# chanzuckerberg/saber

Hardware: AMD Instinct MI355X
Metric: EM slices/sec (1024^2, Hiera-L) (higher is better)
Workload: dtype bf16; 1 GPU; 1024x1024 uint16 EM slice -> prep.prepare -> SAM2 AMG (Hiera-L, cfgAMG defaults: npoints=32, crop_n_layers=2 -> 21 crops, 3072 grid prompts + 9216 m2m refinements, multimask) -> dedup/sort -> uint16 label plane; BASELINE configs[1]; weights=seeded synthetic Hiera-L (no checkpoint offline), slices_per_rank=22, engine_handles_per_gpu=2, parallelism=single GPU

## Files before the change

include/saber_amd.h:

```cpp
#ifndef SABER_AMD_H
#define SABER_AMD_H
#include <stdint.h>

#ifdef __cplusplus
extern "C" {
#endif

typedef struct saber_engine saber_engine;

enum saber_status {
    SABER_OK = 0,
    SABER_ERR_INVALID = -1,
    SABER_ERR_STATE = -2,
    SABER_ERR_HIP = -3,
    SABER_ERR_CAPACITY = -4,
    SABER_ERR_RANGE = -5
};

enum saber_dtype { SABER_U16 = 0, SABER_F32 = 1 };

typedef struct saber_amg_params {
    int points_per_side;
    int points_per_batch;
    float pred_iou_thresh;
// ... 55 lines not shown
#define SABER_WEIGHTS_FP8_E4M3 1
#define SABER_WEIGHTS_MXFP8 2
int saber_engine_set_weight_format(saber_engine* e, int format);

#define SABER_PRECISION_BF16 0
#define SABER_PRECISION_EXACT 1
#define SABER_PRECISION_FP16 2
int saber_engine_set_precision(saber_engine* e, int precision);

int saber_engine_check_finite(saber_engine* e, void* stream);

int saber_engine_set_graphs(saber_engine* e, int enable);
int saber_engine_set_encoder_stream(saber_engine* e, void* stream);
int saber_engine_graph_stats(const saber_engine* e, int* captures, int* replays);

int saber_amg_last_syncs(const saber_engine* e);
int saber_engine_set_device_amg(saber_engine* e, int enable);
int saber_engine_set_iou_pruning(saber_engine* e, int enable);
int saber_engine_set_lowres_cleanup(saber_engine* e, int max_hole_area, int max_sprinkle_area);
int saber_engine_set_multipoint(saber_engine* e, int enable);
int saber_amg_last_pruning(const saber_engine* e, int64_t* pruned, int64_t* m2m_candidates);

int saber_label_plane(saber_engine* e, const uint32_t* bits_dev, const int* order_host, int n, int H, int W,
                      uint16_t* plane_dev, void* stream);

struct saber_window_mask;
int saber_place_window_masks(saber_engine* e, const uint32_t* src_dev, int64_t src_words, const struct saber_window_mask* table_host, int n, int H,
                             int W, uint32_t* out_dev, void* stream);
int saber_window_label_stack(saber_engine* e, const uint32_t* src_dev, int64_t src_words, const struct saber_window_mask* table_host, int n, int first,
                             int count, int H, int W, int elem_bytes, void* out_dev, void* stream);
// ... 88 lines not shown
```

saber_amd/_lib.py:

```python
import ctypes as C
import os
import subprocess

_HERE = os.path.dirname(os.path.abspath(__file__))
LIB_PATH = os.path.join(_HERE, "libsaber_amd.so")
CSRC = os.path.join(_HERE, "csrc")


class SaberAmdError(RuntimeError):
    pass


class SaberRangeError(SaberAmdError):
    """SABER_ERR_RANGE: the engine's overflow sentinel found NaN / inf in the 16-bit arithmetic (include/saber_amd.h:
    saber_engine_check_finite) - with fp16 operands, an activation beyond 65 504.  The call's results are invalid."""


SABER_OK, SABER_ERR_INVALID, SABER_ERR_STATE, SABER_ERR_HIP, SABER_ERR_CAPACITY, SABER_ERR_RANGE = 0, -1, -2, -3, -4, -5


def build(verbose: bool = False) -> str:
    r = subprocess.run(["make", "-C", CSRC, "-j8"], capture_output=True, text=True)
    if r.returncode != 0:
        raise SaberAmdError("building libsaber_amd.so failed:\n" + r.stdout[-4000:] + r.stderr[-4000:])
# ... 57 lines not shown
    "saber_decode_prompts": (_i, [_vp, _i, _vp, _vp, _i, _i, _i, _vp, _vp, _vp, _vp, _vp]),
    "saber_amg_generate": (_i, [_vp, _vp, _i, _i, _i, C.POINTER(AmgParams), _vp, _i, C.POINTER(MaskMeta), C.POINTER(_i), _vp]),
    "saber_amg_postprocess_small_regions": (_i, [_vp, _vp, _i, _i, _i, C.POINTER(MaskMeta), _i, _f, _vp, C.POINTER(_i), _vp]),
    "saber_amg_last_syncs": (_i, [_vp]),
    "saber_engine_set_iou_pruning": (_i, [_vp, _i]),
    "saber_engine_set_lowres_cleanup": (_i, [_vp, _i, _i]),
    "saber_engine_set_multipoint": (_i, [_vp, _i]),
    "saber_engine_set_device_amg": (_i, [_vp, _i]),
    "saber_amg_last_pruning": (_i, [_vp, _vp, _vp]),
    "saber_engine_set_graphs": (_i, [_vp, _i]),
    "saber_engine_set_encoder_stream": (_i, [_vp, _vp]),
    "saber_engine_set_weight_format": (_i, [_vp, _i]),
    "saber_engine_set_precision": (_i, [_vp, _i]),
    "saber_engine_check_finite": (_i, [_vp, _vp]),
    "saber_engine_graph_stats": (_i, [_vp, C.POINTER(_i), C.POINTER(_i)]),
    "saber_label_plane": (_i, [_vp, _vp, C.POINTER(_i), _i, _i, _i, _vp, _vp]),
    "saber_mask_pair_intersections": (_i, [_vp, _vp, _i, _i, _i, _vp, _vp]),
    "saber_place_window_masks": (_i, [_vp, _vp, C.c_int64, C.POINTER(WindowMask), _i, _i, _i, _vp, _vp]),
    "saber_window_label_stack": (_i, [_vp, _vp, C.c_int64, C.POINTER(WindowMask), _i, _i, _i, _i, _i, _i, _vp, _vp]),
    "saber_separate_masks": (_i, [_vp, _vp, _i, _i, _i, _i, _vp, C.POINTER(_i), _vp]),
    "saber_cc_chunk_label": (_i, [_vp, _vp, _i, _i, _i, _vp, _vp, _vp]),
    "saber_cc_seam_pairs": (_i, [_vp, _vp, _vp, _i, _i, C.c_uint32, C.c_uint32, _vp, _i, C.POINTER(_i), _vp]),
    "saber_cc_chunk_roots": (_i, [_vp, _vp, _vp, _i, _i, _i, C.c_uint32, _vp, _i, _vp, _i, C.POINTER(_i), _vp]),
    "saber_cc_chunk_finish": (_i, [_vp, _vp, _vp, _i, _i, _i, _vp, _vp, _i, _vp]),
    "saber_smooth_labels": (_i, [_vp, _vp, _i, _i, _i, _i, C.c_double, _vp, C.POINTER(_i), _vp]),
    "saber_smooth_labels_chunk": (_i, [_vp, _vp, _i, _vp, _i, _vp, _i, _i, _i, _i, _i, _i, _vp, _vp, _i, C.c_double, _vp, C.POINTER(_i), _vp]),
    "saber_smooth_radius": (_i, [C.c_int64, C.c_double, C.POINTER(_i)]),
    "saber_label_max": (_i, [_vp, _vp, _i, C.c_int64, C.POINTER(C.c_uint32), _vp]),
    "saber_label_counts": (_i, [_vp, _vp, _i, _i, _i, _i, _i, _vp, _vp]),
    "saber_gaussian_smoothing_3d": (_i, [_vp, _vp, _i, _i, _i, C.c_double, _vp, _vp]),
# ... 128 lines not shown
```

saber_amd/csrc/amg.hip:

```cpp
#include <algorithm>
#include <array>
#include <cmath>
#include <numeric>

#include "common.h"
#include "engine.h"

#define TRY(x) do { int _r = (x); if (_r != SABER_OK) return _r; } while (0)

struct Cand {
    float box[4];
    float iou, stab;
    float pt[2];
    int crop[4];
    int area;
    size_t bits_slot;
};

static std::vector<int> nms_host(const std::vector<Cand>& c, const std::vector<float>& scores, float thr) {
    const int n = (int)c.size();
    std::vector<int> order(n);
    std::iota(order.begin(), order.end(), 0);
    std::stable_sort(order.begin(), order.end(), [&](int a, int b) { return scores[a] > scores[b]; });
    std::vector<char> sup(n, 0);
// ... 207 lines not shown
        h_pts.resize(n_pts * 2);
        std::vector<float> crop_pts_all(n_pts * 2);
        for (const Grp& gr : groups)
            for (int g = 0; g < gr.G; ++g) {
                const auto& box = crops[c0 + gr.ci + g];
                const int cw = box[2] - box[0], chh = box[3] - box[1];
                for (int iy = 0; iy < gr.gn; ++iy)
                    for (int ix = 0; ix < gr.gn; ++ix) {
                        const float px = (float)(grids[gr.layer][ix] * (double)cw), py = (float)(grids[gr.layer][iy] * (double)chh);
                        const size_t k = gr.pt0 + (size_t)g * gr.np + (size_t)iy * gr.gn + ix;
                        crop_pts_all[2 * k] = px; crop_pts_all[2 * k + 1] = py;
                        h_pts[2 * k] = (px / (float)cw) * 1024.0f;
                        h_pts[2 * k + 1] = (py / (float)chh) * 1024.0f;
                    }
            }
        ENG_HIP(e, hipMemcpyAsync(e->amg_pts, h_pts.data(), sizeof(float) * 2 * n_pts, hipMemcpyHostToDevice, s));
        if (prm->use_m2m) {
            h_pts2.resize(n_cand * 2);
            for (size_t k = 0; k < n_pts; ++k)
                for (int m = 0; m < M; ++m) { h_pts2[2 * (k * M + m)] = h_pts[2 * k]; h_pts2[2 * (k * M + m) + 1] = h_pts[2 * k + 1]; }
            ENG_HIP(e, hipMemcpyAsync(e->amg_pts2, h_pts2.data(), sizeof(float) * 2 * n_cand, hipMemcpyHostToDevice, s));
        }
        for (Grp& gr : groups) {
            const int ci = gr.ci, G = gr.G, np = gr.np, nm = gr.nm;
            float* pts1 = e->amg_pts + 2 * gr.pt0;
            float* low1 = e->amg_low1 + gr.pt0 * (first_raw ? 4 : 1) * 65536;
            float* iou1 = e->amg_iou1 + gr.k0;
            TRY(eng_graphed(e, "dec1," + key_of({ci, np, (long long)(uintptr_t)pts1, G * np, prm->multimask_output, (long long)(uintptr_t)low1, (long long)(uintptr_t)iou1}), s,
                            [&]() { return eng_decode_ex(e, ci, np, pts1, nullptr, G * np, prm->multimask_output, nullptr, 0, 0.f, low1, first_raw, iou1, nullptr, nullptr, s); }));
            for (int g = 0; g < G; ++g) e->slot_shared_valid[ci + g] = 1;
            gr.masks = low1; gr.ious = iou1; gr.plane_mode = first_raw ? 1 : 0;
            if (prm->use_m2m) {
                float* pts2 = e->amg_pts2 + 2 * gr.k0;
                float* low2 = e->amg_low2 + gr.k0 * 4 * 65536;
                float* iou2 = e->amg_iou2 + gr.k0;
                int* sel2 = e->amg_sel + gr.k0;
                TRY(eng_graphed(e, "dec2," + key_of({ci, nm, (long long)(uintptr_t)pts2, G * nm, first_raw, (long long)(uintptr_t)low1, (long long)(uintptr_t)low2, (long long)(uintptr_t)iou2, (long long)(uintptr_t)sel2,
                                                     (long long)(e->iou_prune ? std::lround(prm->pred_iou_thresh * 1e6f) + 1 : 0)}), s,
                                [&]() { return eng_decode_ex(e, ci, nm, pts2, nullptr, G * nm, 0, low1, first_raw, 32.0f, low2, 1, iou2, nullptr, sel2, s, prm->pred_iou_thresh); }));
                for (int g = 0; g < G; ++g) e->slot_embb_valid[ci + g] = 1;
                gr.masks = low2; gr.ious = iou2; gr.plane_mode = 2;
            }
        }
        if (use_dev) {
            const float* iou_all = prm->use_m2m ? e->amg_iou2 : e->amg_iou1;
            std::vector<DevCrop> dcs;
            for (const Grp& gr : groups)
                for (int g = 0; g < gr.G; ++g) {
                    const auto& box = crops[c0 + gr.ci + g];
                    dcs.push_back(DevCrop{{box[0], box[1], box[2], box[3]}, (int)(gr.k0 + (size_t)g * gr.nm), gr.nm, (int)(gr.pt0 + (size_t)g * gr.np), M});
                }
            ENG_HIP(e, hipMemcpyAsync(e->amg_crops_dev, dcs.data(), sizeof(DevCrop) * dcs.size(), hipMemcpyHostToDevice, s));
            size_t dc0 = 0;
            for (const Grp& gr : groups) {
// ... 190 lines not shown
```

saber_amd/csrc/engine.h:

```cpp
#pragma once
#include <hip/hip_runtime.h>
#include <algorithm>
#include <functional>
#include <map>
#include <set>
#include <string>
#include <vector>

#include "../../include/saber_amd.h"
#include "kernels.h"

struct BlockSpec { int din, dout, heads, window, q_stride; };

struct HostTensor { std::vector<int64_t> shape; std::vector<float> data; };

struct LinW { const bf16_t* w = nullptr; const float* b = nullptr; int out = 0, in = 0, ldw = 0; const bf16_t* wpk = nullptr; int wpk_n = 0; const float* wf = nullptr;
              const uint8_t* w8 = nullptr; const uint8_t* sw8 = nullptr; int kp8 = 0, sw_rows = 0; };
struct LnW { const float* g = nullptr; const float* b = nullptr; };

struct BlockW { LnW n1, n2; LinW qkv, proj, fc1, fc2, sc; const bf16_t* mlp_pk = nullptr; };

struct AttnW { LinW q, k, v, o; const bf16_t* pe_proj = nullptr; const bf16_t* img_wT = nullptr; };
struct DecLayerW { AttnW self_attn, t2i, i2t; LnW n1, n2, n3, n4; LinW mlp1, mlp2; };

enum { PC_GEMM = 0, PC_HIERA_ATTN, PC_LAYERNORM, PC_DEC_ATTN, PC_ELEMENTWISE, PC_IMAGE, PC_MASK_POST, PC_DEC_T2I, PC_DEC_I2T, PC_DEC_UPSCALE, PC_GEMM_MX, PC_N };
struct ProfRec { int cls; double flops; double bytes; hipEvent_t a, b; };

struct saber_engine {
    int device = 0;
    std::string trunk;
    int max_images = 1, max_prompts = 64;
    std::string err;
    bool finalized = false;
    int weight_format = 0;
    int precision = 0;
    bool op_f16 = false;
    bool keep_f32 = false;
    void* exact_ws = nullptr;
    void* refine_state = nullptr;
    void* labelstats_ws = nullptr;
    void* sr_ws = nullptr; size_t sr_ws_bytes = 0;
// ... 54 lines not shown
    float* embb = nullptr;
    bf16_t* h2_bf = nullptr;
    std::vector<char> slot_embb_valid;
    std::vector<char> slot_valid, slot_shared_valid;

    float *tok_pe = nullptr, *queries = nullptr, *tq = nullptr, *tk = nullptr;
    bf16_t* t_att = nullptr;
    bf16_t* keys_bf = nullptr;
    bf16_t *fold_q = nullptr, *fold_k = nullptr, *fold_v = nullptr;
    float *fold_cb = nullptr, *t2i_part = nullptr, *t2i_ml = nullptr;
    float *masks4 = nullptr, *hyper_out = nullptr, *iou4 = nullptr;
    bf16_t* hyper_pk = nullptr;
    int* counts_ws = nullptr;
    float* dec_out_masks = nullptr;
    float* dec_out_iou = nullptr;

    float* prep_ws = nullptr; size_t prep_ws_elems = 0; unsigned int* prep_minmax = nullptr;

    float *amg_prep = nullptr; size_t amg_prep_elems = 0;
    int* amg_sel = nullptr; bool amg_m2m_sized = false;
    float *amg_pts = nullptr, *amg_low1 = nullptr, *amg_low2 = nullptr, *amg_iou1 = nullptr, *amg_iou2 = nullptr, *amg_pts2 = nullptr;
    size_t amg_prompts_cap = 0, amg_pts_cap = 0;
    uint32_t* amg_bits = nullptr; size_t amg_bits_words = 0;
    uint32_t* amg_crop_bits = nullptr; size_t amg_crop_words = 0;
    MaskStats* amg_stats = nullptr; int* amg_idx = nullptr; size_t amg_stats_cap = 0;
    int* order_dev = nullptr; size_t order_cap = 0;
    void* win_table_dev = nullptr; size_t win_table_cap = 0;

    bool graphs_on = true;
    std::map<std::string, hipGraphExec_t> graphs;
// ... 54 lines not shown
        if (_st != hipSuccess) { cleanup(); return eng_fail((e), SABER_ERR_HIP, std::string(#call) + ": " + hipGetErrorString(_st)); } \
    } while (0)
#define ENG_K(e, call)                                                   \
    do {                                                                 \
        const char* _m = (call);                                         \
        if (_m) return eng_fail((e), SABER_ERR_INVALID, _m);             \
    } while (0)

int eng_graphed(saber_engine* e, const std::string& key, hipStream_t s, const std::function<int()>& body);
void eng_graphs_flush(saber_engine* e);
int eng_encode(saber_engine* e, const float* img_dev, int H, int W, int channels, const int* crops_host, int n, int slot0, hipStream_t s);
int eng_decode(saber_engine* e, int slot, int per_slot, const float* pts_dev, const int* labels_dev, int n, int multimask,
               const float* mask_in_dev, float mask_clamp, float* out_lowres, float* out_iou, float* out_obj, hipStream_t s);
int eng_decode_ex(saber_engine* e, int slot, int per_slot, const float* pts_dev, const int* labels_dev, int n, int multimask,
                  const float* mask_in_dev, int mask_in_raw4, float mask_clamp, float* out_lowres, int out_raw4, float* out_iou, float* out_obj,
                  int* out_sel, hipStream_t s, float prune_iou_thr = 0.f);
int exact_encode_blocks(saber_engine* e, int n, int slot0, hipStream_t s);
int exact_decode_core(saber_engine* e, int slot0, int per_slot, int p_base, const float* pts, const int* labels, int P, const float* mask_in,
                      float mask_clamp, int mask_in_q0, float* out_obj, float* masks4, hipStream_t s, int n_pts = 1);
int exact_chunk_prompts(const saber_engine* e);
void exact_release(saber_engine* e);
struct UpscalePack {
    std::vector<float> w1, b1;
    std::vector<float> w2, b2;
    std::vector<float> w2p;
};
void saber_pack_upscale(const float* w0, const float* b0, const float* w3, const float* b3, UpscalePack* out);
bf16_t saber_host_f2op(float f, bool f16);
template <typename T> int eng_alloc(saber_engine* e, T** p, size_t count);
int eng_alloc_bytes(saber_engine* e, void** p, size_t bytes);
void eng_free(saber_engine* e, void* p);
// ... 10 lines not shown
```

saber_amd/csrc/engine.hip:

```cpp
#include "engine.h"

#include <algorithm>
#include <cmath>
#include <cstring>
#include <functional>
#include <utility>

#include "common.h"

static thread_local std::string g_create_err;

int eng_fail(saber_engine* e, int code, const std::string& msg) {
    if (e) e->err = msg; else g_create_err = msg;
    return code;
}

int eng_alloc_bytes(saber_engine* e, void** p, size_t bytes) {
    *p = nullptr;
    if (bytes == 0) bytes = 16;
    hipError_t st = hipMalloc(p, bytes);
    if (st != hipSuccess) return eng_fail(e, SABER_ERR_HIP, std::string("hipMalloc(") + std::to_string(bytes) + "): " + hipGetErrorString(st));
    e->allocs.push_back(*p);
    return SABER_OK;
}
// ... 106 lines not shown
extern "C" int saber_engine_set_precision(saber_engine* e, int precision) {
    if (!e) return SABER_ERR_INVALID;
    if (precision != SABER_PRECISION_BF16 && precision != SABER_PRECISION_EXACT && precision != SABER_PRECISION_FP16) return eng_fail(e, SABER_ERR_INVALID, "set_precision: unknown precision");
    if (!e->finalized) {
        if (precision == SABER_PRECISION_EXACT) e->keep_f32 = true;
        else e->op_f16 = precision == SABER_PRECISION_FP16;
    } else {
        if (precision == SABER_PRECISION_EXACT && !e->keep_f32)
            return eng_fail(e, SABER_ERR_STATE, "set_precision: the exact mode needs the fp32 weight copies; request it once before saber_engine_finalize");
        if (precision == SABER_PRECISION_FP16 && !e->op_f16)
            return eng_fail(e, SABER_ERR_STATE, "set_precision: this handle was finalized with bf16 weights; choose SABER_PRECISION_FP16 before saber_engine_finalize");
        if (precision == SABER_PRECISION_BF16 && e->op_f16)
            return eng_fail(e, SABER_ERR_STATE, "set_precision: this handle was finalized with fp16 weights; it runs in SABER_PRECISION_FP16 (or EXACT)");
    }
    e->precision = precision;
    return SABER_OK;
}
extern "C" int saber_engine_set_iou_pruning(saber_engine* e, int enable) {
    if (!e) return SABER_ERR_INVALID;
    if ((bool)enable != e->iou_prune) { e->iou_prune = enable != 0; eng_graphs_flush(e); }
    return SABER_OK;
}
extern "C" int saber_engine_set_lowres_cleanup(saber_engine* e, int max_hole_area, int max_sprinkle_area) {
    if (!e) return SABER_ERR_INVALID;
    if (max_hole_area < 0 || max_hole_area > 65535 || max_sprinkle_area < 0 || max_sprinkle_area > 65535)
        return eng_fail(e, SABER_ERR_INVALID, "set_lowres_cleanup: max_hole_area and max_sprinkle_area must be 0 to 65535");
    e->lowres_hole_area = max_hole_area; e->lowres_sprinkle_area = max_sprinkle_area;
    return SABER_OK;
}
extern "C" int saber_engine_set_multipoint(saber_engine* e, int enable) {
    if (!e) return SABER_ERR_INVALID;
    if (enable && e->max_prompts < 2) return eng_fail(e, SABER_ERR_INVALID, "set_multipoint: the 16-token route needs max_prompts >= 2 (chunks of max_prompts / 2 prompts)");
    e->multipoint = enable != 0;
    return SABER_OK;
}
extern "C" int saber_engine_set_encoder_stream(saber_engine* e, void* stream) {
    if (!e) return SABER_ERR_INVALID;
    if ((hipStream_t)stream != e->enc_stream) { eng_graphs_flush(e); e->enc_stream = (hipStream_t)stream; }
    return SABER_OK;
}
extern "C" int saber_engine_set_graphs(saber_engine* e, int enable) {
    if (!e) return SABER_ERR_INVALID;
    e->graphs_on = enable != 0;
    return SABER_OK;
}
extern "C" int saber_engine_graph_stats(const saber_engine* e, int* captures, int* replays) {
    if (!e) return SABER_ERR_INVALID;
    if (captures) *captures = e->graph_captures;
// ... 39 lines not shown
    *out = e;
    return SABER_OK;
}

extern "C" void saber_engine_destroy(saber_engine* e) {
    if (!e) return;
    (void)hipSetDevice(e->device);
    (void)hipDeviceSynchronize();
    for (auto& kv : e->graphs) (void)hipGraphExecDestroy(kv.second);
    exact_release(e);
    refine_release(e);
    if (e->crops_pin) (void)hipHostFree(e->crops_pin);
    for (hipEvent_t ev : e->crops_ev) if (ev) (void)hipEventDestroy(ev);
    for (hipEvent_t ev : e->enc_ev) if (ev) (void)hipEventDestroy(ev);
    for (void* p : e->allocs) (void)hipFree(p);
    delete e;
}

extern "C" const char* saber_last_error(const saber_engine* e) { return e ? e->err.c_str() : g_create_err.c_str(); }

extern "C" int saber_engine_set_weight(saber_engine* e, const char* name, const float* host, const int64_t* shape, int ndim) {
    if (!e) return SABER_ERR_INVALID;
    if (!name || !host || !shape || ndim < 1 || ndim > 4) return eng_fail(e, SABER_ERR_INVALID, "set_weight: bad argument");
    if (e->finalized) return eng_fail(e, SABER_ERR_STATE, "set_weight after finalize");
    HostTensor t;
    int64_t n = 1;
    for (int i = 0; i < ndim; ++i) { if (shape[i] <= 0) return eng_fail(e, SABER_ERR_INVALID, "set_weight: non-positive dim"); t.shape.push_back(shape[i]); n *= shape[i]; }
    t.data.assign(host, host + n);
    e->host_w[name] = std::move(t);
    return SABER_OK;
// ... 547 lines not shown
            GemmParams g;
            g.A = e->dense_pe_bf; g.lda = 256; g.W = w.w; g.ldw = w.ldw; g.w_kpad = 1; g.M = 4096; g.N = 128; g.K = 256; g.Cb = d; g.ldcb = 128;
            if (const char* m = launch_gemm(g, nullptr)) return eng_fail(e, SABER_ERR_INVALID, m);
            a.pe_proj = d;
            return SABER_OK;
        };
        for (int l = 0; l < 2; ++l) {
            TRY(project(e->dl[l].t2i, e->dl[l].t2i.k));
            TRY(project(e->dl[l].i2t, e->dl[l].i2t.q));
        }
        TRY(project(e->final_attn, e->final_attn.k));
    }
    ENG_HIP(e, hipDeviceSynchronize());
    e->host_w.clear();
    e->finalized = true;
    return SABER_OK;
}

void prof_begin(saber_engine* e, int cls, double flops, double bytes, hipStream_t s) {
    if (!e->prof_on) return;
    while (e->ev_pool.size() < e->ev_used + 2) { hipEvent_t ev; if (hipEventCreate(&ev) != hipSuccess) { e->prof_on = false; return; } e->ev_pool.push_back(ev); }
    ProfRec r; r.cls = cls; r.flops = flops; r.bytes = bytes; r.a = e->ev_pool[e->ev_used++]; r.b = e->ev_pool[e->ev_used++];
    (void)hipEventRecord(r.a, s);
    e->prof.push_back(r);
}
void prof_end(saber_engine* e, hipStream_t s) {
    if (!e->prof_on || e->prof.empty()) return;
    (void)hipEventRecord(e->prof.back().b, s);
}
extern "C" int saber_profile_begin(saber_engine* e) {
// ... 374 lines not shown
    return SABER_OK;
}

static int decode_pick_or_select(saber_engine* e, int P, int multimask, float* out_lowres, float* out_iou, float* raw4_out, int* out_sel, const uint8_t* live,
                                 hipStream_t s) {
    float* oi = out_iou ? out_iou : e->dec_out_iou;
    if (raw4_out) {
        ENG_KP(e, PC_ELEMENTWISE, 0.0, 0.0, launch_mask_pick(raw4_out, e->iou4, P, multimask, oi, out_sel, s, live));
        return SABER_OK;
    }
    float* om = out_lowres ? out_lowres : e->dec_out_masks;
    ENG_KP(e, PC_ELEMENTWISE, 0.0, 0.0, launch_mask_select(e->masks4, e->iou4, P, multimask, om, oi, e->counts_ws, s));
    return SABER_OK;
}

static int decode_chunk(saber_engine* e, int slot0, int per_slot, int p_base, const float* pts, const int* labels, int P, int multimask,
                        const float* mask_in, float mask_clamp, float* out_lowres, float* out_iou, float* out_obj, hipStream_t s,
                        float* raw4_out = nullptr, int* out_sel = nullptr, int mask_in_q0 = -1, float prune_iou_thr = 0.f) {
    if (e->precision == SABER_PRECISION_EXACT) {
        TRY(exact_decode_core(e, slot0, per_slot, p_base, pts, labels, P, mask_in, mask_clamp, mask_in_q0, out_obj, raw4_out ? raw4_out : e->masks4, s, e->decode_n_pts));
        return decode_pick_or_select(e, P, multimask, out_lowres, out_iou, raw4_out, out_sel, nullptr, s);
    }
    const int K = e->decode_n_pts;
    if (K != 1 && !e->multipoint)
        return eng_fail(e, SABER_ERR_STATE, "prompts of several points (clicks, boxes) are decoded in the exact precision mode only: the bf16 kernels are built for 8 decoder tokens per prompt");
    const int R = K != 1 ? 16 : 8, nh = R / 8, nvalid = 7 + K;
    if (R == 16) {
        if (K < 2 || K > 9) return eng_fail(e, SABER_ERR_INVALID, "decode: the 16-token route takes 2..9 points per prompt");
        if (2 * P > e->max_prompts) return eng_fail(e, SABER_ERR_INVALID, "decode: a 16-token chunk holds at most max_prompts / 2 prompts");
    }
    const int PT = P * R;
    const size_t o256 = (size_t)slot0 * 4096 * 256;
    const int slot_last = slot0 + (p_base + P - 1) / per_slot;
    const XMap slots{(int64_t)4096 * 256, per_slot, p_base};
    const XMap per_prompt{(int64_t)4096 * 256, 1, 0};
    const float kScale = 0.25f * 1.4426950408889634f;
    int split = 1;
    while (split < 8 && nh * P * split < 512) split *= 2;
    if (R == 16) ENG_KP(e, PC_ELEMENTWISE, 0.0, 0.0, launch_prompt_tokens16(pts, labels, P, K, e->pw, e->tok_pe, s));
    else ENG_KP(e, PC_ELEMENTWISE, 0.0, 0.0, launch_prompt_tokens(pts, labels, P, e->pw, e->tok_pe, s));
    ENG_HIP(e, hipMemcpyAsync(e->queries, e->tok_pe, sizeof(float) * PT * 256, hipMemcpyDeviceToDevice, s));
    e->dec_tok_rows = R;
    const bf16_t* X;
    XMap xm;
    XBuild xb;
    const XBuild* build = nullptr;
    const bool no_build = R == 16 || getenv("SABER_AMD_XBUILD") == nullptr;
    if (mask_in == nullptr) {
        for (int sl = slot0 + p_base / per_slot; sl <= slot_last; ++sl) TRY(ensure_shared(e, sl, s));
        X = e->src0_bf + o256; xm = slots;
    } else if (no_build) {
        ENG_KP(e, PC_ELEMENTWISE, 0.0, (double)P * (65536.0 * 4 + 4096.0 * 256 * 2), launch_mask_embed_src(mask_in, P, e->emb + o256, slots, e->dense_pe, e->mw, nullptr, e->keys_bf, nullptr, mask_clamp, s, mask_in_q0));
        X = e->keys_bf; xm = per_prompt;
    } else {
        for (int sl = slot0 + p_base / per_slot; sl <= slot_last; ++sl) TRY(ensure_embb(e, sl, s));
        ENG_KP(e, PC_ELEMENTWISE, 0.0, (double)P * (65536.0 * 4 + 4096.0 * 16 * 2), launch_mask_hidden(mask_in, P, e->mw, e->h2_bf, mask_clamp, s, mask_in_q0));
        xb.embb = e->embb + o256; xb.map = slots; xb.h2 = e->h2_bf; xb.w3 = e->mw.w3;
        build = &xb;
        X = nullptr; xm = per_prompt;
    }

    auto lin = [](const LinW& l) { TokLin t; t.w = l.w; t.b = l.b; t.ldw = l.ldw; t.n = l.out; t.wpk = l.wpk; t.npk = l.wpk_n; return t; };
    auto lnw = [](const LnW& l) { TokLn t; t.g = l.g; t.b = l.b; return t; };
    auto base = [&]() { TokSeg g; g.P = P; g.queries = e->queries; g.tok_pe = e->tok_pe; g.kscale = kScale; return g; };
    auto with_t2i = [&](TokSeg& g, const AttnW& a) { g.do_t2i = 1; g.t2i_q = lin(a.q); g.t2i_kT = a.img_wT; g.tq_out = e->tq; g.fold_q = e->fold_q; };
    auto with_self = [&](TokSeg& g, const DecLayerW& w, int first) {
        g.do_self = 1; g.self_first = first; g.sa_q = lin(w.self_attn.q); g.sa_k = lin(w.self_attn.k); g.sa_v = lin(w.self_attn.v); g.sa_o = lin(w.self_attn.o); g.ln1 = lnw(w.n1);
    };
    auto with_att_out = [&](TokSeg& g, const AttnW& a, const LnW& ln) { g.t_att = e->t_att; g.att_o = lin(a.o); g.att_ln = lnw(ln); g.att_eps = 1e-5f; };
    auto with_mlp_i2t = [&](TokSeg& g, const DecLayerW& w) {
        g.do_mlp = 1; g.mlp1 = lin(w.mlp1); g.mlp2 = lin(w.mlp2); g.mlp1_pk = w.mlp1.wpk; g.mlp2_pk = w.mlp2.wpk; g.ln3 = lnw(w.n3);
        g.i2t_k = lin(w.i2t.k); g.i2t_v = lin(w.i2t.v); g.i2t_qT = w.i2t.img_wT; g.i2t_qb = w.i2t.q.b; g.i2t_o = w.i2t.o.w;
        g.tk_out = e->tk; g.fold_k = e->fold_k; g.fold_cb = e->fold_cb; g.fold_v = e->fold_v;
    };
    const double tflops = 2.0 * PT * 256.0;
    const double xflops = 4.0 * (8 * R) * 4096.0 * 256 * P;
    auto run_tokens = [&](const TokSeg& g, double cols) -> int {
        if (R == 16) ENG_KP(e, PC_DEC_ATTN, tflops * cols, 0.0, launch_dec_tokens16(g, nvalid, s));
        else ENG_KP(e, PC_DEC_ATTN, tflops * cols, 0.0, launch_dec_tokens(g, s));
        return SABER_OK;
    };
    auto run_t2i = [&](const AttnW& a) -> int {
        ENG_KP(e, PC_DEC_T2I, xflops, (double)P * 4096 * 256 * 2 * nh,
               launch_dec_t2i(X, XMap{xm.stride, nh * xm.div, nh * xm.off}, a.pe_proj, e->fold_q, e->tq, kScale, e->t2i_part, e->t2i_ml, nh * P, split, a.v.w, a.v.b, e->t_att, s, build));
        return SABER_OK;
    };
    auto run_i2t = [&](const DecLayerW& w) -> int {
        if (R == 16) ENG_KP(e, PC_DEC_I2T, xflops, (double)P * 4096 * 256 * 4, launch_dec_i2t16(X, xm, w.i2t.pe_proj, e->fold_k, e->tk, kScale, e->fold_cb, e->fold_v, w.i2t.o.b, w.n4.g, w.n4.b, 1e-5f, e->keys_bf, P, nvalid, s));
        else ENG_KP(e, PC_DEC_I2T, xflops, (double)P * 4096 * 256 * 4, launch_dec_i2t(X, xm, w.i2t.pe_proj, e->fold_k, e->tk, kScale, e->fold_cb, e->fold_v, w.i2t.o.b, w.n4.g, w.n4.b, 1e-5f, e->keys_bf, P, s, build));
        X = e->keys_bf; xm = per_prompt; build = nullptr;
        return SABER_OK;
    };
    {
        TokSeg g = base(); with_self(g, e->dl[0], 1); with_t2i(g, e->dl[0].t2i);
        TRY(run_tokens(g, 4 * 256 + 128 + 128));
    }
    TRY(run_t2i(e->dl[0].t2i));
    {
        TokSeg g = base(); with_att_out(g, e->dl[0].t2i, e->dl[0].n2); with_mlp_i2t(g, e->dl[0]); with_self(g, e->dl[1], 0); with_t2i(g, e->dl[1].t2i);
        TRY(run_tokens(g, 128 + 4096 + 4 * 128 + 4 * 256 + 256));
    }
    TRY(run_i2t(e->dl[0]));
    TRY(run_t2i(e->dl[1].t2i));
    {
        TokSeg g = base(); with_att_out(g, e->dl[1].t2i, e->dl[1].n2); with_mlp_i2t(g, e->dl[1]); with_t2i(g, e->final_attn);
        TRY(run_tokens(g, 128 + 4096 + 4 * 128 + 256));
    }
    TRY(run_i2t(e->dl[1]));
    TRY(run_t2i(e->final_attn));
    {
        TokSeg g = base(); with_att_out(g, e->final_attn, e->final_ln);
        g.do_heads = 1;
        for (int l = 0; l < 3; ++l) { g.iou[l] = lin(e->iou_head[l]); g.obj[l] = lin(e->obj_head[l]); g.hyper[l] = lin(e->hyper[l]); }
        g.iou4 = e->iou4; g.obj_out = out_obj; g.hyper_out = e->hyper_out;
        TRY(run_tokens(g, 128 + 6 * 512.0 / R));
    }
    ENG_KP(e, PC_ELEMENTWISE, 0.0, 0.0, launch_nonfinite_scan(e->iou4, (int64_t)P * 4, e->nonfinite + 1, s));
    ENG_KP(e, PC_ELEMENTWISE, 0.0, 0.0, launch_hyper_pack(e->hyper_out, P, e->hyper_pk, e->nonfinite + 1, s));
    const uint8_t* live = nullptr;
    if (prune_iou_thr > 0.f && raw4_out && !multimask && e->iou_prune) {
        ENG_KP(e, PC_ELEMENTWISE, 0.0, 0.0, launch_iou_live_flags(e->iou4, P, prune_iou_thr, e->live, e->prune_counters, s));
        live = e->live;
    }
    ENG_KP(e, PC_DEC_UPSCALE, (double)P * 2.0 * (4096.0 * 256 * 256 + 16384.0 * 64 * 128 + 65536.0 * 32 * 4), (double)P * (4096.0 * 256 * 2 + 4 * 65536.0 * 4),
           launch_dec_upscale(X, e->dc1.w, e->dc1.b, e->up_ln.g, e->up_ln.b, e->dc2p, e->dc2.b, e->fs1 + (size_t)slot0 * 16384 * 64,
                              e->fs0 + (size_t)slot0 * 65536 * 32, XMap{0, per_slot, p_base}, e->hyper_out, e->hyper_pk, raw4_out ? raw4_out : e->masks4, P, s, live,
                              getenv("SABER_AMD_ALL_PLANES") ? nullptr : e->iou4, multimask, e->nonfinite + 2));
    return decode_pick_or_select(e, P, multimask, out_lowres, out_iou, raw4_out, out_sel, live, s);
}

int eng_decode(saber_engine* e, int slot, int per_slot, const float* pts_dev, const int* labels_dev, int n, int multimask,
               const float* mask_in_dev, float mask_clamp, float* out_lowres, float* out_iou, float* out_obj, hipStream_t s) {
    return eng_decode_ex(e, slot, per_slot, pts_dev, labels_dev, n, multimask, mask_in_dev, 0, mask_clamp, out_lowres, 0, out_iou, out_obj, nullptr, s);
}
int eng_decode_ex(saber_engine* e, int slot, int per_slot, const float* pts_dev, const int* labels_dev, int n, int multimask,
                  const float* mask_in_dev, int mask_in_raw4, float mask_clamp, float* out_lowres, int out_raw4, float* out_iou, float* out_obj,
                  int* out_sel, hipStream_t s, float prune_iou_thr) {
    if (!e->finalized) return eng_fail(e, SABER_ERR_STATE, "engine not finalized");
    if (!pts_dev || n < 0 || per_slot < 0) return eng_fail(e, SABER_ERR_INVALID, "decode: bad argument");
    if (per_slot == 0 || per_slot > n) per_slot = n > 0 ? n : 1;
    const int nslots = n > 0 ? (n + per_slot - 1) / per_slot : 1;
    for (int sl = slot; sl < slot + nslots; ++sl)
        if (sl < 0 || sl >= e->max_images || !e->slot_valid[sl]) return eng_fail(e, SABER_ERR_STATE, "decode: slot holds no encoded image; call saber_encode first");
    const int M = multimask ? 3 : 1;
    const int K = e->decode_n_pts;
    const int chunk = e->precision == SABER_PRECISION_EXACT ? std::max(1, exact_chunk_prompts(e) * 8 / (7 + K))
                      : K > 1 && e->multipoint ? std::max(1, e->max_prompts / 2)
                                               : e->max_prompts;
    e->dec_tok_rows = 8;
    for (int p0 = 0; p0 < n; p0 += chunk) {
        const int P = std::min(chunk, n - p0);
        const float* min_ = !mask_in_dev ? nullptr : mask_in_raw4 ? mask_in_dev : mask_in_dev + (size_t)p0 * 65536;
        TRY(decode_chunk(e, slot, per_slot, p0, pts_dev + 2 * (size_t)p0 * K, labels_dev ? labels_dev + (size_t)p0 * K : nullptr, P, multimask,
                         min_, mask_clamp,
                         out_lowres && !out_raw4 ? out_lowres + (size_t)p0 * M * 65536 : nullptr, out_iou ? out_iou + (size_t)p0 * M : nullptr,
                         out_obj ? out_obj + p0 : nullptr, s, out_raw4 ? out_lowres + (size_t)p0 * 4 * 65536 : nullptr,
                         out_sel ? out_sel + p0 : nullptr, mask_in_dev && mask_in_raw4 ? p0 : -1, prune_iou_thr));
    }
    ENG_HIP(e, hipGetLastError());
    return SABER_OK;
}

extern "C" int saber_decode_points(saber_engine* e, int slot, const float* pts_dev, const int* labels_dev, int n, int multimask,
                                   const float* mask_in_dev, float* out_lowres_dev, float* out_iou_dev, float* out_obj_dev, void* stream) {
    if (!e) return SABER_ERR_INVALID;
    ENG_DEVICE(e);
    return eng_decode(e, slot, 0, pts_dev, labels_dev, n, multimask, mask_in_dev, 0.f, out_lowres_dev, out_iou_dev, out_obj_dev, (hipStream_t)stream);
}

extern "C" int saber_decode_prompts(saber_engine* e, int slot, const float* pts_dev, const int* labels_dev, int n, int points_per_prompt, int multimask,
                                    const float* mask_in_dev, float* out_lowres_dev, float* out_iou_dev, float* out_obj_dev, void* stream) {
    if (!e) return SABER_ERR_INVALID;
// ... 58 lines not shown
```

saber_amd/engine.py:

```python
import ctypes as C
import os
from typing import Dict, List, Optional, Sequence

import numpy as np
import torch

from . import _lib
from .model_config import get_config
from .weights import seeded_weights, load_checkpoint

SABER_U16, SABER_F32 = 0, 1


def _ptr(t: Optional[torch.Tensor]):
    return None if t is None else C.c_void_p(t.data_ptr())


def _stream():
    return C.c_void_p(torch.cuda.current_stream().cuda_stream)


class Engine:

    def __init__(self, trunk: str = "large", device: int = 0, weights: Optional[Dict[str, np.ndarray]] = None,
# ... 668 lines not shown

    def last_pruning(self):
        a, b = C.c_int64(0), C.c_int64(0)
        self._check(self.lib.saber_amg_last_pruning(self.h, C.byref(a), C.byref(b)))
        return a.value, b.value

    def set_graphs(self, enable: bool):
        self._check(self.lib.saber_engine_set_graphs(self.h, int(bool(enable))))

    def graph_stats(self):
        import ctypes as C
        c, r = C.c_int(0), C.c_int(0)
        self._check(self.lib.saber_engine_graph_stats(self.h, C.byref(c), C.byref(r)))
        return c.value, r.value

    def profile_begin(self):
        self._check(self.lib.saber_profile_begin(self.h))

    def profile_end(self) -> dict:
        n = len(_lib.PROFILE_CLASSES)
        arr = (_lib.ProfileClass * n)()
        self._check(self.lib.saber_profile_end(self.h, arr, n))
        return {name: {"launches": int(arr[i].launches), "ms": float(arr[i].ms), "flops": float(arr[i].flops), "bytes": float(arr[i].bytes)}
                for i, name in enumerate(_lib.PROFILE_CLASSES)}

    def encoder_flops(self) -> float:
        return float(self.lib.saber_encoder_flops(self.h))


def _check_cleanup_areas(who: str, max_hole_area, max_sprinkle_area):
# ... 53 lines not shown
```

Measured before the change: 7.819 slices/s.

## Cache prompt-only decoder stage across calls for repeated AMG grid prompts

Adds a device-side cache keyed on the grid point coordinates that stores prompt tokens, initial queries, the layer-0 self-attention output and the t2i query projections. When the same grid appears again, decoding reuses these and skips the point upload and the image-independent first token stage. Entries are invalidated on precision, multipoint or finalize changes and evicted LRU, which adds device memory and host-side memcmp lookups. Graph keys now include the cache entry so captured graphs stay consistent.

```diff
diff --git a/include/saber_amd.h b/include/saber_amd.h
--- a/include/saber_amd.h
+++ b/include/saber_amd.h
@@ -93,6 +93,9 @@
 int saber_engine_set_encoder_stream(saber_engine* e, void* stream);
 int saber_engine_graph_stats(const saber_engine* e, int* captures, int* replays);
 
+int saber_engine_prompt_cache_stats(const saber_engine* e, long long* hits, long long* misses);
+int saber_engine_prompt_cache_info(const saber_engine* e, int* entries, long long* bytes);
+
 int saber_amg_last_syncs(const saber_engine* e);
 int saber_engine_set_device_amg(saber_engine* e, int enable);
 int saber_engine_set_iou_pruning(saber_engine* e, int enable);
diff --git a/saber_amd/_lib.py b/saber_amd/_lib.py
--- a/saber_amd/_lib.py
+++ b/saber_amd/_lib.py
@@ -95,6 +95,8 @@
     "saber_engine_set_precision": (_i, [_vp, _i]),
     "saber_engine_check_finite": (_i, [_vp, _vp]),
     "saber_engine_graph_stats": (_i, [_vp, C.POINTER(_i), C.POINTER(_i)]),
+    "saber_engine_prompt_cache_stats": (_i, [_vp, C.POINTER(C.c_longlong), C.POINTER(C.c_longlong)]),
+    "saber_engine_prompt_cache_info": (_i, [_vp, C.POINTER(_i), C.POINTER(C.c_longlong)]),
     "saber_label_plane": (_i, [_vp, _vp, C.POINTER(_i), _i, _i, _i, _vp, _vp]),
     "saber_mask_pair_intersections": (_i, [_vp, _vp, _i, _i, _i, _vp, _vp]),
     "saber_place_window_masks": (_i, [_vp, _vp, C.c_int64, C.POINTER(WindowMask), _i, _i, _i, _vp, _vp]),
diff --git a/saber_amd/csrc/amg.hip b/saber_amd/csrc/amg.hip
--- a/saber_amd/csrc/amg.hip
+++ b/saber_amd/csrc/amg.hip
@@ -245,20 +245,44 @@
                         h_pts[2 * k + 1] = (py / (float)chh) * 1024.0f;
                     }
             }
-        ENG_HIP(e, hipMemcpyAsync(e->amg_pts, h_pts.data(), sizeof(float) * 2 * n_pts, hipMemcpyHostToDevice, s));
         if (prm->use_m2m) {
             h_pts2.resize(n_cand * 2);
             for (size_t k = 0; k < n_pts; ++k)
                 for (int m = 0; m < M; ++m) { h_pts2[2 * (k * M + m)] = h_pts[2 * k]; h_pts2[2 * (k * M + m) + 1] = h_pts[2 * k + 1]; }
-            ENG_HIP(e, hipMemcpyAsync(e->amg_pts2, h_pts2.data(), sizeof(float) * 2 * n_cand, hipMemcpyHostToDevice, s));
-        }
-        for (Grp& gr : groups) {
+        }
+        const bool pc_on = eng_prompt_cache_on(e);
+        const long long pc_tag = ((long long)H << 32) | (long long)W;
+        const unsigned long long pc_pin = e->pcache_clock;
+        std::vector<int> set1(groups.size(), -1), set2(groups.size(), -1);
+        std::vector<char> fill1(groups.size(), 0), fill2(groups.size(), 0);
+        bool up1 = !pc_on, up2 = !pc_on;
+        if (pc_on)
+            for (size_t gi = 0; gi < groups.size(); ++gi) {
+                const Grp& gr = groups[gi];
+                bool nf = false;
+                set1[gi] = eng_prompt_cache_lookup(e, h_pts.data() + 2 * gr.pt0, gr.G * gr.np, pc_tag, pc_pin, &nf);
+                fill1[gi] = nf; up1 = up1 || nf || set1[gi] < 0;
+                if (prm->use_m2m) {
+                    set2[gi] = eng_prompt_cache_lookup(e, h_pts2.data() + 2 * gr.k0, gr.G * gr.nm, pc_tag, pc_pin, &nf);
+                    fill2[gi] = nf; up2 = up2 || nf || set2[gi] < 0;
+                }
+            }
+        if (up1) ENG_HIP(e, hipMemcpyAsync(e->amg_pts, h_pts.data(), sizeof(float) * 2 * n_pts, hipMemcpyHostToDevice, s));
+        if (prm->use_m2m && up2) ENG_HIP(e, hipMemcpyAsync(e->amg_pts2, h_pts2.data(), sizeof(float) * 2 * n_cand, hipMemcpyHostToDevice, s));
+        for (size_t gi = 0; gi < groups.size(); ++gi) {
+            if (fill1[gi]) TRY(eng_prompt_cache_fill(e, set1[gi], e->amg_pts + 2 * groups[gi].pt0, s));
+            if (fill2[gi]) TRY(eng_prompt_cache_fill(e, set2[gi], e->amg_pts2 + 2 * groups[gi].k0, s));
+        }
+        for (size_t gi = 0; gi < groups.size(); ++gi) {
+            Grp& gr = groups[gi];
             const int ci = gr.ci, G = gr.G, np = gr.np, nm = gr.nm;
             float* pts1 = e->amg_pts + 2 * gr.pt0;
             float* low1 = e->amg_low1 + gr.pt0 * (first_raw ? 4 : 1) * 65536;
             float* iou1 = e->amg_iou1 + gr.k0;
-            TRY(eng_graphed(e, "dec1," + key_of({ci, np, (long long)(uintptr_t)pts1, G * np, prm->multimask_output, (long long)(uintptr_t)low1, (long long)(uintptr_t)iou1}), s,
-                            [&]() { return eng_decode_ex(e, ci, np, pts1, nullptr, G * np, prm->multimask_output, nullptr, 0, 0.f, low1, first_raw, iou1, nullptr, nullptr, s); }));
+            const int ps1 = set1[gi], ps2 = set2[gi];
+            const long long pa1 = ps1 >= 0 ? (long long)(uintptr_t)e->pcache[ps1].base : 0, pa2 = ps2 >= 0 ? (long long)(uintptr_t)e->pcache[ps2].base : 0;
+            TRY(eng_graphed(e, "dec1," + key_of({ci, np, (long long)(uintptr_t)pts1, G * np, prm->multimask_output, (long long)(uintptr_t)low1, (long long)(uintptr_t)iou1, ps1, pa1}), s,
+                            [&]() { return eng_decode_ex(e, ci, np, pts1, nullptr, G * np, prm->multimask_output, nullptr, 0, 0.f, low1, first_raw, iou1, nullptr, nullptr, s, 0.f, ps1); }));
             for (int g = 0; g < G; ++g) e->slot_shared_valid[ci + g] = 1;
             gr.masks = low1; gr.ious = iou1; gr.plane_mode = first_raw ? 1 : 0;
             if (prm->use_m2m) {
@@ -267,8 +291,8 @@
                 float* iou2 = e->amg_iou2 + gr.k0;
                 int* sel2 = e->amg_sel + gr.k0;
                 TRY(eng_graphed(e, "dec2," + key_of({ci, nm, (long long)(uintptr_t)pts2, G * nm, first_raw, (long long)(uintptr_t)low1, (long long)(uintptr_t)low2, (long long)(uintptr_t)iou2, (long long)(uintptr_t)sel2,
-                                                     (long long)(e->iou_prune ? std::lround(prm->pred_iou_thresh * 1e6f) + 1 : 0)}), s,
-                                [&]() { return eng_decode_ex(e, ci, nm, pts2, nullptr, G * nm, 0, low1, first_raw, 32.0f, low2, 1, iou2, nullptr, sel2, s, prm->pred_iou_thresh); }));
+                                                     (long long)(e->iou_prune ? std::lround(prm->pred_iou_thresh * 1e6f) + 1 : 0), ps2, pa2}), s,
+                                [&]() { return eng_decode_ex(e, ci, nm, pts2, nullptr, G * nm, 0, low1, first_raw, 32.0f, low2, 1, iou2, nullptr, sel2, s, prm->pred_iou_thresh, ps2); }));
                 for (int g = 0; g < G; ++g) e->slot_embb_valid[ci + g] = 1;
                 gr.masks = low2; gr.ious = iou2; gr.plane_mode = 2;
             }
diff --git a/saber_amd/csrc/engine.h b/saber_amd/csrc/engine.h
--- a/saber_amd/csrc/engine.h
+++ b/saber_amd/csrc/engine.h
@@ -25,6 +25,20 @@
 
 enum { PC_GEMM = 0, PC_HIERA_ATTN, PC_LAYERNORM, PC_DEC_ATTN, PC_ELEMENTWISE, PC_IMAGE, PC_MASK_POST, PC_DEC_T2I, PC_DEC_I2T, PC_DEC_UPSCALE, PC_GEMM_MX, PC_N };
 struct ProfRec { int cls; double flops; double bytes; hipEvent_t a, b; };
+
+struct PromptSet {
+    std::vector<float> pts;
+    long long tag = 0;
+    int n = 0;
+    bool op_f16 = false;
+    unsigned long long gen = 0;
+    bool filled = false;
+    unsigned long long last_use = 0;
+    void* base = nullptr; size_t cap = 0;
+    float *tok_pe = nullptr, *queries = nullptr, *tq = nullptr;
+    bf16_t* fold_q = nullptr;
+};
+enum { PCACHE_MAX_ENTRIES = 16, PCACHE_MAX_PROMPTS = 1 << 16, PCACHE_BYTES_PER_PROMPT = 8 * 256 * 4 * 2 + 8 * 128 * 4 + 64 * 256 * 2, PCACHE_DEBUG_OFF = 524288 };
 
 struct saber_engine {
     int device = 0;
@@ -109,6 +123,10 @@
     int* counts_ws = nullptr;
     float* dec_out_masks = nullptr;
     float* dec_out_iou = nullptr;
+    std::vector<PromptSet> pcache;
+    unsigned long long pcache_gen = 1;
+    unsigned long long pcache_clock = 0;
+    long long pcache_hits = 0, pcache_misses = 0;
 
     float* prep_ws = nullptr; size_t prep_ws_elems = 0; unsigned int* prep_minmax = nullptr;
 
@@ -193,7 +211,11 @@
                const float* mask_in_dev, float mask_clamp, float* out_lowres, float* out_iou, float* out_obj, hipStream_t s);
 int eng_decode_ex(saber_engine* e, int slot, int per_slot, const float* pts_dev, const int* labels_dev, int n, int multimask,
                   const float* mask_in_dev, int mask_in_raw4, float mask_clamp, float* out_lowres, int out_raw4, float* out_iou, float* out_obj,
-                  int* out_sel, hipStream_t s, float prune_iou_thr = 0.f);
+                  int* out_sel, hipStream_t s, float prune_iou_thr = 0.f,
+                  int prompt_set = -1);
+bool eng_prompt_cache_on(const saber_engine* e);
+int eng_prompt_cache_lookup(saber_engine* e, const float* pts_host, int n, long long tag, unsigned long long pin, bool* need_fill);
+int eng_prompt_cache_fill(saber_engine* e, int set, const float* pts_dev, hipStream_t s);
 int exact_encode_blocks(saber_engine* e, int n, int slot0, hipStream_t s);
 int exact_decode_core(saber_engine* e, int slot0, int per_slot, int p_base, const float* pts, const int* labels, int P, const float* mask_in,
                       float mask_clamp, int mask_in_q0, float* out_obj, float* masks4, hipStream_t s, int n_pts = 1);
diff --git a/saber_amd/csrc/engine.hip b/saber_amd/csrc/engine.hip
--- a/saber_amd/csrc/engine.hip
+++ b/saber_amd/csrc/engine.hip
@@ -144,6 +144,7 @@
             return eng_fail(e, SABER_ERR_STATE, "set_precision: this handle was finalized with fp16 weights; it runs in SABER_PRECISION_FP16 (or EXACT)");
     }
     e->precision = precision;
+    ++e->pcache_gen;
     return SABER_OK;
 }
 extern "C" int saber_engine_set_iou_pruning(saber_engine* e, int enable) {
@@ -162,6 +163,7 @@
     if (!e) return SABER_ERR_INVALID;
     if (enable && e->max_prompts < 2) return eng_fail(e, SABER_ERR_INVALID, "set_multipoint: the 16-token route needs max_prompts >= 2 (chunks of max_prompts / 2 prompts)");
     e->multipoint = enable != 0;
+    ++e->pcache_gen;
     return SABER_OK;
 }
 extern "C" int saber_engine_set_encoder_stream(saber_engine* e, void* stream) {
@@ -231,6 +233,7 @@
     for (hipEvent_t ev : e->crops_ev) if (ev) (void)hipEventDestroy(ev);
     for (hipEvent_t ev : e->enc_ev) if (ev) (void)hipEventDestroy(ev);
     for (void* p : e->allocs) (void)hipFree(p);
+    for (PromptSet& ps : e->pcache) if (ps.base) (void)hipFree(ps.base);
     delete e;
 }
 
@@ -808,6 +811,7 @@
     ENG_HIP(e, hipDeviceSynchronize());
     e->host_w.clear();
     e->finalized = true;
+    ++e->pcache_gen;
     return SABER_OK;
 }
 
@@ -1212,9 +1216,105 @@
     return SABER_OK;
 }
 
+static TokLin tok_lin(const LinW& l) { TokLin t; t.w = l.w; t.b = l.b; t.ldw = l.ldw; t.n = l.out; t.wpk = l.wpk; t.npk = l.wpk_n; return t; }
+static TokLn tok_ln(const LnW& l) { TokLn t; t.g = l.g; t.b = l.b; return t; }
+static const float kDecScale = 0.25f * 1.4426950408889634f;
+static int run_s0(saber_engine* e, int P, float* queries, const float* tok_pe, float* tq, bf16_t* fold_q, hipStream_t s) {
+    TokSeg g; g.P = P; g.queries = queries; g.tok_pe = tok_pe; g.kscale = kDecScale;
+    const DecLayerW& w = e->dl[0];
+    g.do_self = 1; g.self_first = 1; g.sa_q = tok_lin(w.self_attn.q); g.sa_k = tok_lin(w.self_attn.k); g.sa_v = tok_lin(w.self_attn.v); g.sa_o = tok_lin(w.self_attn.o); g.ln1 = tok_ln(w.n1);
+    g.do_t2i = 1; g.t2i_q = tok_lin(w.t2i.q); g.t2i_kT = w.t2i.img_wT; g.tq_out = tq; g.fold_q = fold_q;
+    ENG_KP(e, PC_DEC_ATTN, 2.0 * P * 8 * 256.0 * (4 * 256 + 128 + 128), 0.0, launch_dec_tokens(g, s));
+    return SABER_OK;
+}
+
+bool eng_prompt_cache_on(const saber_engine* e) {
+    if (e->precision == SABER_PRECISION_EXACT || e->decode_n_pts != 1) return false;
+    if (g_saber_debug_flags & PCACHE_DEBUG_OFF) return false;
+    const char* off = getenv("SABER_AMD_NO_PROMPT_CACHE");
+    return !(off && off[0] && off[0] != '0');
+}
+static void pcache_release(saber_engine* e, PromptSet& ps) {
+    if (ps.base) {
+        eng_graphs_flush(e);
+        (void)hipFree(ps.base);
+    }
+    ps.base = nullptr; ps.cap = 0; ps.filled = false; ps.n = 0; ps.pts.clear();
+}
+int eng_prompt_cache_lookup(saber_engine* e, const float* pts_host, int n, long long tag, unsigned long long pin, bool* need_fill) {
+    *need_fill = false;
+    if (n <= 0 || n > PCACHE_MAX_PROMPTS || !pts_host) return -1;
+    for (size_t i = 0; i < e->pcache.size(); ++i) {
+        PromptSet& ps = e->pcache[i];
+        if (ps.n != n || ps.tag != tag || ps.gen != e->pcache_gen || ps.op_f16 != e->op_f16 || !ps.base || ps.pts.size() != (size_t)2 * n) continue;
+        if (memcmp(ps.pts.data(), pts_host, sizeof(float) * 2 * n) != 0) continue;
+        ps.last_use = ++e->pcache_clock;
+        *need_fill = !ps.filled;
+        if (ps.filled) ++e->pcache_hits;
+        return (int)i;
+    }
+    ++e->pcache_misses;
+    int at = -1;
+    for (size_t i = 0; i < e->pcache.size() && at < 0; ++i)
+        if (e->pcache[i].gen != e->pcache_gen && e->pcache[i].last_use <= pin) at = (int)i;
+    if (at < 0) {
+        if (e->pcache.size() < (size_t)PCACHE_MAX_ENTRIES) { e->pcache.emplace_back(); at = (int)e->pcache.size() - 1; }
+        else
+            for (size_t i = 0; i < e->pcache.size(); ++i)
+                if (e->pcache[i].last_use <= pin && (at < 0 || e->pcache[i].last_use < e->pcache[at].last_use)) at = (int)i;
+    }
+    if (at < 0) return -1;
+    PromptSet& ps = e->pcache[at];
+    if (ps.cap < (size_t)n) {
+        pcache_release(e, ps);
+        if (hipMalloc(&ps.base, (size_t)n * PCACHE_BYTES_PER_PROMPT) != hipSuccess) { (void)hipGetLastError(); ps.base = nullptr; ps.gen = 0; return -1; }
+        ps.cap = (size_t)n;
+    }
+    char* b = reinterpret_cast<char*>(ps.base);
+    ps.tok_pe = reinterpret_cast<float*>(b);
+    ps.queries = reinterpret_cast<float*>(b + ps.cap * 8192);
+    ps.tq = reinterpret_cast<float*>(b + ps.cap * 16384);
+    ps.fold_q = reinterpret_cast<bf16_t*>(b + ps.cap * 20480);
+    ps.pts.assign(pts_host, pts_host + (size_t)2 * n);
+    ps.n = n; ps.tag = tag; ps.op_f16 = e->op_f16; ps.gen = e->pcache_gen; ps.filled = false;
+    ps.last_use = ++e->pcache_clock;
+    *need_fill = true;
+    return at;
+}
+int eng_prompt_cache_fill(saber_engine* e, int set, const float* pts_dev, hipStream_t s) {
+    if (set < 0 || set >= (int)e->pcache.size() || !pts_dev) return eng_fail(e, SABER_ERR_INVALID, "prompt cache: bad entry");
+    PromptSet& ps = e->pcache[set];
+    if (ps.filled) return SABER_OK;
+    for (int p0 = 0; p0 < ps.n; p0 += e->max_prompts) {
+        const int P = std::min(e->max_prompts, ps.n - p0);
+        float* tok_pe = ps.tok_pe + (size_t)p0 * 2048;
+        float* queries = ps.queries + (size_t)p0 * 2048;
+        ENG_KP(e, PC_ELEMENTWISE, 0.0, 0.0, launch_prompt_tokens(pts_dev + 2 * (size_t)p0, nullptr, P, e->pw, tok_pe, s));
+        ENG_HIP(e, hipMemcpyAsync(queries, tok_pe, sizeof(float) * (size_t)P * 2048, hipMemcpyDeviceToDevice, s));
+        TRY(run_s0(e, P, queries, tok_pe, ps.tq + (size_t)p0 * 1024, ps.fold_q + (size_t)p0 * 64 * 256, s));
+    }
+    ps.filled = true;
+    return SABER_OK;
+}
+extern "C" int saber_engine_prompt_cache_stats(const saber_engine* e, long long* hits, long long* misses) {
+    if (!e) return SABER_ERR_INVALID;
+    if (hits) *hits = e->pcache_hits;
+    if (misses) *misses = e->pcache_misses;
+    return SABER_OK;
+}
+extern "C" int saber_engine_prompt_cache_info(const saber_engine* e, int* entries, long long* bytes) {
+    if (!e) return SABER_ERR_INVALID;
+    long long b = 0;
+    int n = 0;
+    for (const PromptSet& ps : e->pcache) if (ps.base) { ++n; b += (long long)ps.cap * PCACHE_BYTES_PER_PROMPT; }
+    if (entries) *entries = n;
+    if (bytes) *bytes = b;
+    return SABER_OK;
+}
+
 static int decode_chunk(saber_engine* e, int slot0, int per_slot, int p_base, const float* pts, const int* labels, int P, int multimask,
                         const float* mask_in, float mask_clamp, float* out_lowres, float* out_iou, float* out_obj, hipStream_t s,
-                        float* raw4_out = nullptr, int* out_sel = nullptr, int mask_in_q0 = -1, float prune_iou_thr = 0.f) {
+                        float* raw4_out = nullptr, int* out_sel = nullptr, int mask_in_q0 = -1, float prune_iou_thr = 0.f, const PromptSet* pc = nullptr) {
     if (e->precision == SABER_PRECISION_EXACT) {
         TRY(exact_decode_core(e, slot0, per_slot, p_base, pts, labels, P, mask_in, mask_clamp, mask_in_q0, out_obj, raw4_out ? raw4_out : e->masks4, s, e->decode_n_pts));
         return decode_pick_or_select(e, P, multimask, out_lowres, out_iou, raw4_out, out_sel, nullptr, s);
@@ -1232,12 +1332,16 @@
     const int slot_last = slot0 + (p_base + P - 1) / per_slot;
     const XMap slots{(int64_t)4096 * 256, per_slot, p_base};
     const XMap per_prompt{(int64_t)4096 * 256, 1, 0};
-    const float kScale = 0.25f * 1.4426950408889634f;
+    const float kScale = kDecScale;
     int split = 1;
     while (split < 8 && nh * P * split < 512) split *= 2;
+    if (pc && (R != 8 || labels || !pc->filled || p_base + P > pc->n)) return eng_fail(e, SABER_ERR_STATE, "decode: the prompt-set cache entry does not hold this chunk");
+    const float* tok_pe = pc ? pc->tok_pe + (size_t)p_base * 2048 : e->tok_pe;
+    const float* tq0 = pc ? pc->tq + (size_t)p_base * 1024 : e->tq;
+    const bf16_t* fold_q0 = pc ? pc->fold_q + (size_t)p_base * 64 * 256 : e->fold_q;
     if (R == 16) ENG_KP(e, PC_ELEMENTWISE, 0.0, 0.0, launch_prompt_tokens16(pts, labels, P, K, e->pw, e->tok_pe, s));
-    else ENG_KP(e, PC_ELEMENTWISE, 0.0, 0.0, launch_prompt_tokens(pts, labels, P, e->pw, e->tok_pe, s));
-    ENG_HIP(e, hipMemcpyAsync(e->queries, e->tok_pe, sizeof(float) * PT * 256, hipMemcpyDeviceToDevice, s));
+    else if (!pc) ENG_KP(e, PC_ELEMENTWISE, 0.0, 0.0, launch_prompt_tokens(pts, labels, P, e->pw, e->tok_pe, s));
+    ENG_HIP(e, hipMemcpyAsync(e->queries, pc ? pc->queries + (size_t)p_base * 2048 : e->tok_pe, sizeof(float) * PT * 256, hipMemcpyDeviceToDevice, s));
     e->dec_tok_rows = R;
     const bf16_t* X;
     XMap xm;
@@ -1258,9 +1362,9 @@
         X = nullptr; xm = per_prompt;
     }
 
-    auto lin = [](const LinW& l) { TokLin t; t.w = l.w; t.b = l.b; t.ldw = l.ldw; t.n = l.out; t.wpk = l.wpk; t.npk = l.wpk_n; return t; };
-    auto lnw = [](const LnW& l) { TokLn t; t.g = l.g; t.b = l.b; return t; };
-    auto base = [&]() { TokSeg g; g.P = P; g.queries = e->queries; g.tok_pe = e->tok_pe; g.kscale = kScale; return g; };
+    auto lin = tok_lin;
+    auto lnw = tok_ln;
+    auto base = [&]() { TokSeg g; g.P = P; g.queries = e->queries; g.tok_pe = tok_pe; g.kscale = kScale; return g; };
     auto with_t2i = [&](TokSeg& g, const AttnW& a) { g.do_t2i = 1; g.t2i_q = lin(a.q); g.t2i_kT = a.img_wT; g.tq_out = e->tq; g.fold_q = e->fold_q; };
     auto with_self = [&](TokSeg& g, const DecLayerW& w, int first) {
         g.do_self = 1; g.self_first = first; g.sa_q = lin(w.self_attn.q); g.sa_k = lin(w.self_attn.k); g.sa_v = lin(w.self_attn.v); g.sa_o = lin(w.self_attn.o); g.ln1 = lnw(w.n1);
@@ -1278,9 +1382,9 @@
         else ENG_KP(e, PC_DEC_ATTN, tflops * cols, 0.0, launch_dec_tokens(g, s));
         return SABER_OK;
     };
-    auto run_t2i = [&](const AttnW& a) -> int {
+    auto run_t2i = [&](const AttnW& a, const bf16_t* fold_q, const float* tq) -> int {
         ENG_KP(e, PC_DEC_T2I, xflops, (double)P * 4096 * 256 * 2 * nh,
-               launch_dec_t2i(X, XMap{xm.stride, nh * xm.div, nh * xm.off}, a.pe_proj, e->fold_q, e->tq, kScale, e->t2i_part, e->t2i_ml, nh * P, split, a.v.w, a.v.b, e->t_att, s, build));
+               launch_dec_t2i(X, XMap{xm.stride, nh * xm.div, nh * xm.off}, a.pe_proj, fold_q, tq, kScale, e->t2i_part, e->t2i_ml, nh * P, split, a.v.w, a.v.b, e->t_att, s, build));
         return SABER_OK;
     };
     auto run_i2t = [&](const DecLayerW& w) -> int {
@@ -1289,23 +1393,23 @@
         X = e->keys_bf; xm = per_prompt; build = nullptr;
         return SABER_OK;
     };
-    {
+    if (R == 16) {
         TokSeg g = base(); with_self(g, e->dl[0], 1); with_t2i(g, e->dl[0].t2i);
         TRY(run_tokens(g, 4 * 256 + 128 + 128));
-    }
-    TRY(run_t2i(e->dl[0].t2i));
+    } else if (!pc) TRY(run_s0(e, P, e->queries, e->tok_pe, e->tq, e->fold_q, s));
+    TRY(run_t2i(e->dl[0].t2i, fold_q0, tq0));
     {
         TokSeg g = base(); with_att_out(g, e->dl[0].t2i, e->dl[0].n2); with_mlp_i2t(g, e->dl[0]); with_self(g, e->dl[1], 0); with_t2i(g, e->dl[1].t2i);
         TRY(run_tokens(g, 128 + 4096 + 4 * 128 + 4 * 256 + 256));
     }
     TRY(run_i2t(e->dl[0]));
-    TRY(run_t2i(e->dl[1].t2i));
+    TRY(run_t2i(e->dl[1].t2i, e->fold_q, e->tq));
     {
         TokSeg g = base(); with_att_out(g, e->dl[1].t2i, e->dl[1].n2); with_mlp_i2t(g, e->dl[1]); with_t2i(g, e->final_attn);
         TRY(run_tokens(g, 128 + 4096 + 4 * 128 + 256));
     }
     TRY(run_i2t(e->dl[1]));
-    TRY(run_t2i(e->final_attn));
+    TRY(run_t2i(e->final_attn, e->fold_q, e->tq));
     {
         TokSeg g = base(); with_att_out(g, e->final_attn, e->final_ln);
         g.do_heads = 1;
@@ -1333,9 +1437,15 @@
 }
 int eng_decode_ex(saber_engine* e, int slot, int per_slot, const float* pts_dev, const int* labels_dev, int n, int multimask,
                   const float* mask_in_dev, int mask_in_raw4, float mask_clamp, float* out_lowres, int out_raw4, float* out_iou, float* out_obj,
-                  int* out_sel, hipStream_t s, float prune_iou_thr) {
+                  int* out_sel, hipStream_t s, float prune_iou_thr, int prompt_set) {
     if (!e->finalized) return eng_fail(e, SABER_ERR_STATE, "engine not finalized");
     if (!pts_dev || n < 0 || per_slot < 0) return eng_fail(e, SABER_ERR_INVALID, "decode: bad argument");
+    const PromptSet* pc = nullptr;
+    if (prompt_set >= 0) {
+        if (prompt_set >= (int)e->pcache.size() || e->pcache[prompt_set].n != n || !e->pcache[prompt_set].filled || !eng_prompt_cache_on(e))
+            return eng_fail(e, SABER_ERR_STATE, "decode: the prompt-set cache entry does not hold this call's prompts");
+        pc = &e->pcache[prompt_set];
+    }
     if (per_slot == 0 || per_slot > n) per_slot = n > 0 ? n : 1;
     const int nslots = n > 0 ? (n + per_slot - 1) / per_slot : 1;
     for (int sl = slot; sl < slot + nslots; ++sl)
@@ -1353,7 +1463,7 @@
                          min_, mask_clamp,
                          out_lowres && !out_raw4 ? out_lowres + (size_t)p0 * M * 65536 : nullptr, out_iou ? out_iou + (size_t)p0 * M : nullptr,
                          out_obj ? out_obj + p0 : nullptr, s, out_raw4 ? out_lowres + (size_t)p0 * 4 * 65536 : nullptr,
-                         out_sel ? out_sel + p0 : nullptr, mask_in_dev && mask_in_raw4 ? p0 : -1, prune_iou_thr));
+                         out_sel ? out_sel + p0 : nullptr, mask_in_dev && mask_in_raw4 ? p0 : -1, prune_iou_thr, pc));
     }
     ENG_HIP(e, hipGetLastError());
     return SABER_OK;
diff --git a/saber_amd/engine.py b/saber_amd/engine.py
--- a/saber_amd/engine.py
+++ b/saber_amd/engine.py
@@ -706,6 +706,18 @@
         self._check(self.lib.saber_engine_graph_stats(self.h, C.byref(c), C.byref(r)))
         return c.value, r.value
 
+    def prompt_cache_stats(self):
+        import ctypes as C
+        h, m = C.c_longlong(0), C.c_longlong(0)
+        self._check(self.lib.saber_engine_prompt_cache_stats(self.h, C.byref(h), C.byref(m)))
+        return h.value, m.value
+
+    def prompt_cache_info(self):
+        import ctypes as C
+        n, b = C.c_int(0), C.c_longlong(0)
+        self._check(self.lib.saber_engine_prompt_cache_info(self.h, C.byref(n), C.byref(b)))
+        return n.value, b.value
+
     def profile_begin(self):
         self._check(self.lib.saber_profile_begin(self.h))
 
```

Result: no change. 7.850 slices/s, median of 6 (+0.4%).
